# aviadlevis/bhnerf

Hardware: AMD Instinct MI355X
Metric: train ray-samples/sec, 128x128x64-sample image-plane recovery (higher is better)
Workload: dtype bf16

## Files before the change

bhnerf_amd/csrc/fused_bwd128.hip:

```cpp
#include <type_traits>
#include "bwd_common.h"

namespace {

constexpr int MT = 4, KS = 8, TB = 2048;
constexpr int IMG = 32768;
constexpr int OFF_GA = 0, OFF_H = 2 * IMG, OFF_E = 4 * IMG;
constexpr int ENC_IMG = 8192;
constexpr int OFF_DOUT = OFF_E + 2 * ENC_IMG;
constexpr int OFF_DPK = OFF_DOUT + 512;
constexpr int OFF_W0 = OFF_DPK + 256;
constexpr int OFF_B0 = OFF_W0 + 8192;
constexpr int LDS_BYTES = OFF_B0 + 512;
constexpr int CB = (KS + 2) * 1024;
constexpr int SLAB_TILES = 65;
constexpr int SLAB_FLOATS128 = SLAB_TILES * 1024;
constexpr int CPF = 3;

typedef PolBF16 Pol;
typedef Pol::frag frag;

DEVI frag lds_row(const char *smem, unsigned off) { return *reinterpret_cast<const frag *>(smem + off); }
DEVI void lds_put(char *smem, unsigned off, const frag &f) { *reinterpret_cast<frag *>(smem + off) = f; }

DEVI frag tr2(const char *smem, unsigned off_a, unsigned off_b) {
    typedef s16x4 __attribute__((address_space(3))) * lds_v4;
    typedef short s16x8 __attribute__((ext_vector_type(8)));
    const s16x4 lo = __builtin_amdgcn_ds_read_tr16_b64_v4i16((lds_v4)(smem + off_a));
    const s16x4 hi = __builtin_amdgcn_ds_read_tr16_b64_v4i16((lds_v4)(smem + off_b));
    const s16x8 v = __builtin_shufflevector(lo, hi, 0, 1, 2, 3, 4, 5, 6, 7);
    return __builtin_bit_cast(frag, v);
}

DEVI u32x4 make_rsrc(const char *p) {
    const unsigned long long u = reinterpret_cast<unsigned long long>(p);
    const unsigned lo = __builtin_amdgcn_readfirstlane((unsigned)u), hi = __builtin_amdgcn_readfirstlane((unsigned)(u >> 32));
    return u32x4{lo, hi & 0xffffu, 0x7fffffffu, 0x00020000u};
}
#pragma clang diagnostic push
#pragma clang diagnostic ignored "-Winline-asm"
DEVI void dma_piece(const u32x4 &rs, unsigned soff, unsigned lds, unsigned voff) {
    asm volatile("s_mov_b32 m0, %0\n\ts_nop 0\n\tbuffer_load_dwordx4 %1, %2, %3 offen nt lds" ::"s"(lds), "v"(voff), "s"(rs), "s"(soff) : "memory", "m0");
}
#pragma clang diagnostic pop

DEVI unsigned keep_where_nz(unsigned g, unsigned h) {
    typedef short i16x2 __attribute__((ext_vector_type(2)));
    const unsigned sgn = h + 0x7fff7fffu;
    return g & __builtin_bit_cast(unsigned, __builtin_bit_cast(i16x2, sgn) >> (i16x2){15, 15});
}


template <int DEPTH, int SKIPL>
__global__ __launch_bounds__(256) __attribute__((amdgpu_waves_per_eu(1, 1))) void bwd128_kernel(BwdArgs A) {
    static_assert(DEPTH >= 2 && DEPTH <= 4, "14 accumulator tiles per wave at depth 4");
    extern __shared__ __attribute__((aligned(16))) char smem[];
    const FusedArgs &a = A.f;
    clock_stamp(a.clk, BHN_CLK_CHAIN, 0);
    const int tid = threadIdx.x, lane = tid & 63;
    const int wv = __builtin_amdgcn_readfirstlane(tid >> 6);
    const int wi = wv >> 1, wj = wv & 1;
    const int pl = lane & 31, hh = lane >> 5;

    unsigned rowb[2];
    {
        const int swz = ((pl & 3) << 2) | (((pl >> 2) & 3) ^ (pl & 2));
#pragma unroll
        for (int pi = 0; pi < 2; ++pi) rowb[pi] = 256u * (32 * (2 * wj + pi) + pl) + 16u * ((hh ^ swz) & 15);
    }
    const int tg = lane >> 4, tcg = tg & 1, tkh = tg >> 1, tq = (lane & 15) >> 2, tp = lane & 3;
    auto tr_first = [&](int T) -> unsigned {
        const int lc = 2 * tcg + (tp >> 1), swa = (tq << 2) | ((2 * tkh) ^ (tq & 2));
        return 256u * (8 * tkh + tq) + 16u * (((4 * T) ^ lc ^ swa) & 15) + 8u * (tp & 1);
    };
    auto tr_second = [&](int T) -> unsigned {
        const int lc = 2 * tcg + (tp >> 1), swb = (tq << 2) | ((2 * tkh + 1) ^ (tq & 2));
        return 256u * (8 * tkh + tq + 4) + 16u * (((4 * T) ^ lc ^ swb) & 15) + 8u * (tp & 1);
    };
    const unsigned trA_m0 = tr_first(2 * wi), trB_m0 = tr_second(2 * wi), trA_m1 = tr_first(2 * wi + 1), trB_m1 = tr_second(2 * wi + 1);
    const unsigned trA_n0 = tr_first(2 * wj), trB_n0 = tr_second(2 * wj), trA_n1 = tr_first(2 * wj + 1), trB_n1 = tr_second(2 * wj + 1);
    const unsigned trA_w = tr_first(wv), trB_w = tr_second(wv);
    const unsigned trA_me = tr_first(2 * wi + wj), trB_me = tr_second(2 * wi + wj);
    const unsigned trE = 64u * (8 * tkh + tq) + 32u * tcg + 8u * tp;

    const unsigned voffH = 2048u * ((((lane & 15) >> 2) ^ (lane >> 4)) & 3) + 64u * (((lane & 3) ^ wv ^ ((lane >> 4) & 2)) & 3) + 16u * (lane >> 4);
    const unsigned voffE = 16u * ((lane >> 2) & 3) + 64u * (lane & 3) + 256u * (lane >> 4);
    const unsigned lds0 = __builtin_amdgcn_readfirstlane((unsigned)reinterpret_cast<unsigned long long>(smem));

    const long long nquads = A.t.NQ >> 2;
    const long long h_stride = A.t.lin_stride;
    auto dma_h = [&](int l, long long Q, int hb) {
        const u32x4 rs = make_rsrc(A.tape + A.t.h_lin + (long long)l * h_stride + Q * (4ll * MT * TB));
#pragma unroll
        for (int t = 0; t < 8; ++t) {
            const int pb = t >> 1, kk = wv + 4 * (t & 1), k = wv + 4 * t;
            dma_piece(rs, (unsigned)(pb * (MT * TB) + 256 * kk), lds0 + OFF_H + hb * IMG + 1024 * k, voffH);
        }
    };
    auto h_rsrc = [&](int l, long long Q) { return make_rsrc(A.tape + A.t.h_lin + (long long)l * h_stride + Q * (4ll * MT * TB)); };
    auto dma_h_piece = [&](const u32x4 &rs, int hb, int t) {
        const int pb = t >> 1, kk = wv + 4 * (t & 1), k = wv + 4 * t;
        dma_piece(rs, (unsigned)(pb * (MT * TB) + 256 * kk), lds0 + OFF_H + hb * IMG + 1024 * k, voffH);
    };
    auto dma_enc = [&](long long Q, int eb) {
        const u32x4 rs = make_rsrc(A.tape + A.t.enc_off + Q * (4ll * TB));
#pragma unroll
        for (int t = 0; t < 2; ++t) {
            const int e = wv + 4 * t, pb = e >> 1, half = e & 1;
            dma_piece(rs, (unsigned)(pb * TB + 1024 * half), lds0 + OFF_E + eb * ENC_IMG + 1024 * e, voffE);
        }
    };
    const float *dout_g = reinterpret_cast<const float *>(A.tape + A.t.dout_off);
    auto point_dout = [&](long long Q) -> float { return dout_g[(4 * Q + wv) * 32 + pl]; };
    auto put_dout = [&](float d) {
        if (lane < 32) reinterpret_cast<float *>(smem + OFF_DOUT)[32 * wv + pl] = d;
    };
    const unsigned *maskd_g = reinterpret_cast<const unsigned *>(A.tape + A.t.maskd_off);
    auto load_maskd = [&](long long Qx, unsigned (&mw)[2]) {
#pragma unroll
        for (int pi = 0; pi < 2; ++pi) mw[pi] = maskd_g[((4 * Qx + 2 * wj + pi) * 2 + wi) * 64 + lane];
    };
    const __amdgpu_buffer_rsrc_t wrs = __builtin_amdgcn_make_buffer_rsrc(
        const_cast<char *>(a.packed + a.bwd_off + (size_t)(2 * wi) * CB), 0, 0x7fffffff, 0x00020000);
    auto load_w1 = [&](int l, int mi, int ks) -> frag {
        return __builtin_bit_cast(frag, __builtin_amdgcn_raw_buffer_load_b128(wrs, lane * 16, ((l - 1) * MT + mi) * CB + ks * 1024, 0));
    };
    auto load_w = [&](int l, frag (&wf)[2][KS]) {
#pragma unroll
        for (int mi = 0; mi < 2; ++mi)
#pragma unroll
            for (int ks = 0; ks < KS; ++ks) wf[mi][ks] = load_w1(l, mi, ks);
    };
    auto use_w = [&](frag (&wf)[2][KS]) {
#pragma unroll
        for (int mi = 0; mi < 2; ++mi)
#pragma unroll
            for (int ks = 0; ks < KS; ks += 4) asm volatile("" : "+v"(wf[mi][ks]), "+v"(wf[mi][ks + 1]), "+v"(wf[mi][ks + 2]), "+v"(wf[mi][ks + 3]));
    };
    auto drain_and_barrier = [&]() {
        asm volatile("s_waitcnt vmcnt(0) lgkmcnt(0)" ::: "memory");
        __builtin_amdgcn_s_barrier();
        asm volatile("" ::: "memory");
    };

    f32x16 acc[DEPTH - 1][4], acc_e, acc0;
#pragma unroll
    for (int l = 0; l < DEPTH - 1; ++l)
#pragma unroll
        for (int t = 0; t < 4; ++t) { const f32x16 z = {}; acc[l][t] = z; }
    { const f32x16 z = {}; acc_e = z; acc0 = z; }
    float bsum[DEPTH - 1];
#pragma unroll
    for (int l = 0; l < DEPTH - 1; ++l) bsum[l] = 0.f;
    float bout = 0.f;

    auto chain_mma = [&](const frag (&wf)[2][KS], unsigned ga_in, int pi, f32x16 (&c)[2], auto &&side) {
        { const f32x16 z = {}; c[0] = z; c[1] = z; }
        frag bq[CPF + 1];
#pragma unroll
        for (int i = 0; i < CPF; ++i) bq[i] = lds_row(smem, ga_in + (rowb[pi] ^ (32u * i)));
#pragma unroll
        for (int ks = 0; ks < KS; ++ks) {
            if (ks + CPF < KS) bq[(ks + CPF) % (CPF + 1)] = lds_row(smem, ga_in + (rowb[pi] ^ (32u * (ks + CPF))));
            __builtin_amdgcn_sched_barrier(0);
            c[0] = Pol::mma(wf[0][ks], bq[ks % (CPF + 1)], c[0]);
            c[1] = Pol::mma(wf[1][ks], bq[ks % (CPF + 1)], c[1]);
            side(ks);
            __builtin_amdgcn_sched_barrier(0);
        }
        asm volatile("" : "+v"(c[0]), "+v"(c[1]));
    };
    u32x4 ps_hv, ps_hvn, ps_o;
    auto post_off = [&](int pi, int jp) -> unsigned { return rowb[pi] ^ (16u * (4 * (2 * wi + (jp >> 1)) + 2 * (jp & 1))); };
    auto post_begin = [&](int pi, unsigned h_img) { ps_hvn = __builtin_bit_cast(u32x4, lds_row(smem, h_img + post_off(pi, 0))); };
    auto post_slice = [&](const f32x16 (&c)[2], int pi, unsigned h_img, unsigned ga_out, int j) {
        const int mi = j >> 2, s2 = (j >> 1) & 1, half = j & 1;
        if (half == 0) ps_hv = ps_hvn;
        else if (j + 1 < 8) ps_hvn = __builtin_bit_cast(u32x4, lds_row(smem, h_img + post_off(pi, (j + 1) >> 1)));
#pragma unroll
        for (int d = 2 * half; d < 2 * half + 2; ++d) ps_o[d] = keep_where_nz(Pol::pack_a(c[mi][8 * s2 + 2 * d], c[mi][8 * s2 + 2 * d + 1]), ps_hv[d]);
        if (half == 1) lds_put(smem, ga_out + post_off(pi, j >> 1), __builtin_bit_cast(frag, ps_o));
    };
    auto dw_phase = [&](auto enc_tag, unsigned ga_img, unsigned h_img, unsigned e_img, f32x16 (&t)[4], f32x16 &te, float &bs, auto &&side) {
        constexpr bool ENC = decltype(enc_tag)::value;
        struct KF { frag a0, a1, b0, b1, ae, be; };
        auto fetch = [&](int k) {
            KF f;
            const unsigned ko = 4096u * k;
            f.a0 = tr2(smem, ga_img + trA_m0 + ko, ga_img + trB_m0 + ko);
            f.a1 = tr2(smem, ga_img + trA_m1 + ko, ga_img + trB_m1 + ko);
            f.b0 = tr2(smem, h_img + trA_n0 + ko, h_img + trB_n0 + ko);
            f.b1 = tr2(smem, h_img + trA_n1 + ko, h_img + trB_n1 + ko);
            f.ae = tr2(smem, ga_img + trA_me + ko, ga_img + trB_me + ko);
            if constexpr (ENC) f.be = tr2(smem, e_img + trE + 1024u * k, e_img + trE + 1024u * k + 256u);
            else f.be = f.b0;
            return f;
        };
        KF cur = fetch(0);
#pragma unroll
        for (int k = 0; k < 8; ++k) {
            __builtin_amdgcn_sched_barrier(0);
            t[0] = Pol::mma(cur.a0, cur.b0, t[0]);
            t[1] = Pol::mma(cur.a0, cur.b1, t[1]);
            t[2] = Pol::mma(cur.a1, cur.b0, t[2]);
            t[3] = Pol::mma(cur.a1, cur.b1, t[3]);
            if constexpr (ENC) te = Pol::mma(cur.ae, cur.be, te);
            else bs = Pol::sum8(cur.ae, bs);
            if (k + 1 < 8) cur = fetch(k + 1);
            side(k);
            __builtin_amdgcn_sched_barrier(0);
        }
    };
    auto dw0_phase = [&](unsigned ga_img, unsigned e_img, auto &&side) {
        frag af = tr2(smem, ga_img + trA_w, ga_img + trB_w);
        frag be = tr2(smem, e_img + trE, e_img + trE + 256u);
#pragma unroll
        for (int k = 0; k < 8; ++k) {
            frag afn = af, ben = be;
            if (k + 1 < 8) {
                const unsigned ko = 4096u * (k + 1);
                afn = tr2(smem, ga_img + trA_w + ko, ga_img + trB_w + ko);
                ben = tr2(smem, e_img + trE + 1024u * (k + 1), e_img + trE + 1024u * (k + 1) + 256u);
            }
            __builtin_amdgcn_sched_barrier(0);
            acc0 = Pol::mma(af, be, acc0);
            side(k);
            __builtin_amdgcn_sched_barrier(0);
            af = afn; be = ben;
        }
    };
    auto front = [&](const unsigned (&mw)[2], unsigned ga_out) {
#pragma unroll
        for (int pi = 0; pi < 2; ++pi) {
            const float dvp = reinterpret_cast<const float *>(smem + OFF_DOUT)[32 * (2 * wj + pi) + pl];
            const Pol::bf16x2 d2 = {(__bf16)dvp, (__bf16)dvp};
            const unsigned dd = __builtin_bit_cast(unsigned, d2);
#pragma unroll
            for (int mi = 0; mi < 2; ++mi) {
                const unsigned code = mi ? mw[pi] >> 16 : mw[pi];
#pragma unroll
                for (int s2 = 0; s2 < 2; ++s2) {
                    u32x4 o;
#pragma unroll
                    for (int d = 0; d < 4; ++d) {
                        const int lo = (int)(code << (31 - (4 * s2 + d))) >> 31, hi = (int)(code << (31 - (8 + 4 * s2 + d))) >> 31;
                        o[d] = dd & (((unsigned)lo & 0xffffu) | ((unsigned)hi & 0xffff0000u));
                    }
                    lds_put(smem, ga_out + (rowb[pi] ^ (16u * (4 * (2 * wi + mi) + 2 * s2))), __builtin_bit_cast(frag, o));
                }
            }
        }
    };

    for (int i = tid; i < 8192 / 16; i += 256)
        reinterpret_cast<u32x4 *>(smem + OFF_W0)[i] = reinterpret_cast<const u32x4 *>(a.packed + a.fwd_off)[i];
    if (tid < 128) reinterpret_cast<float *>(smem + OFF_B0)[tid] = reinterpret_cast<const float *>(a.packed + a.bias_off)[tid];
    auto make_h1 = [&](unsigned e_img, unsigned h_out) {
        frag eb[2][2], wa[2][2];
#pragma unroll
        for (int pi = 0; pi < 2; ++pi)
#pragma unroll
            for (int ks = 0; ks < 2; ++ks) eb[pi][ks] = lds_row(smem, e_img + 64u * (32 * (2 * wj + pi) + pl) + 16u * (2 * ks + hh));
#pragma unroll
        for (int mi = 0; mi < 2; ++mi)
#pragma unroll
            for (int ks = 0; ks < 2; ++ks) wa[mi][ks] = lds_row(smem, OFF_W0 + 1024u * (2 * (2 * wi + mi) + ks) + 16u * lane);
#pragma unroll
        for (int mi = 0; mi < 2; ++mi) {
            const f32x16 b0 = bias_acc(reinterpret_cast<const float *>(smem + OFF_B0), 2 * wi + mi, hh);
#pragma unroll
            for (int pi = 0; pi < 2; ++pi) {
                f32x16 t = b0;
                t = Pol::mma(wa[mi][0], eb[pi][0], t);
                t = Pol::mma(wa[mi][1], eb[pi][1], t);
                asm volatile("" : "+v"(t));
                frag o[2];
                unsigned unused = 0;
#pragma unroll
                for (int r = 0; r < 16; r += 2) Pol::relu_pair(o[r >> 3], (r & 7) >> 1, r >> 1, t[r], t[r + 1], unused);
#pragma unroll
                for (int s2 = 0; s2 < 2; ++s2) lds_put(smem, h_out + (rowb[pi] ^ (16u * (4 * (2 * wi + mi) + 2 * s2))), o[s2]);
            }
        }
    };

    long long Q = blockIdx.x;
    frag wf[2][KS];
    float dnext = 0.f;
    int eb = 0;
    unsigned mnext[2] = {0u, 0u};
    if (Q < nquads) {
        dma_h(DEPTH - 1, Q, 1);
        dma_enc(Q, 0);
        dnext = point_dout(Q);
        load_maskd(Q, mnext);
        load_w(DEPTH - 1, wf);
        use_w(wf);
        if (lane < 32) bout += dnext;
        put_dout(dnext);
        drain_and_barrier();
        front(mnext, OFF_GA + 0 * IMG);
        drain_and_barrier();
    }
    for (; Q < nquads; Q += gridDim.x) {
#pragma unroll
        for (int l = 0; l < DEPTH - 1; ++l) asm volatile("" : "+a"(acc[l][0]), "+a"(acc[l][1]), "+a"(acc[l][2]), "+a"(acc[l][3]));
        asm volatile("" : "+a"(acc_e), "+a"(acc0));
        const bool has_next = Q + gridDim.x < nquads;
        const long long Qn = has_next ? Q + gridDim.x : Q;
        const unsigned e_img = OFF_E + eb * ENC_IMG;
#pragma unroll
        for (int l = DEPTH - 1; l >= 1; --l) {
            const int gi = (DEPTH - 1 - l) & 1, hi = (DEPTH - l) & 1;
            const unsigned ga_in = OFF_GA + gi * IMG, ga_out = OFF_GA + (gi ^ 1) * IMG, h_img = OFF_H + hi * IMG;
            const u32x4 rs_h = h_rsrc(l - 1 >= 2 ? l - 1 : 2, Q);
            if (l == 2) make_h1(e_img, OFF_H + (hi ^ 1) * IMG);
            if (l == 1) { dnext = point_dout(Qn); load_maskd(Qn, mnext); }
            f32x16 c0[2], c1[2];
            chain_mma(wf, ga_in, 0, c0, [&](int ks) { if (l - 1 >= 2) dma_h_piece(rs_h, hi ^ 1, ks); });
            post_begin(0, h_img);
            chain_mma(wf, ga_in, 1, c1, [&](int ks) { post_slice(c0, 0, h_img, ga_out, ks); });
            post_begin(1, h_img);
            const int ln = (l - 1 >= 1) ? l - 1 : DEPTH - 1;
            auto side_dw = [&](int k) {
                post_slice(c1, 1, h_img, ga_out, k);
                if (k < 4) {
#pragma unroll
                    for (int mi = 0; mi < 2; ++mi) { wf[mi][2 * k] = load_w1(ln, mi, 2 * k); wf[mi][2 * k + 1] = load_w1(ln, mi, 2 * k + 1); }
                }
            };
            if (l == SKIPL) dw_phase(std::true_type{}, ga_in, h_img, e_img, acc[l - 1], acc_e, bsum[l - 1], side_dw);
            else dw_phase(std::false_type{}, ga_in, h_img, e_img, acc[l - 1], acc_e, bsum[l - 1], side_dw);
            use_w(wf);
            if (l == 1) {
                asm volatile("" : "+v"(dnext));
                const float d = has_next ? dnext : 0.f;
                if (lane < 32) bout += d;
                put_dout(d);
            }
            drain_and_barrier();
        }
        {
            const int gi0 = (DEPTH - 1) & 1, hfree = (DEPTH - 1) & 1;
            const u32x4 rs_h = h_rsrc(DEPTH - 1, Qn);
            dma_enc(Qn, eb ^ 1);
            dw0_phase(OFF_GA + gi0 * IMG, e_img, [&](int k) { dma_h_piece(rs_h, hfree, k); });
            front(mnext, OFF_GA + 0 * IMG);
            drain_and_barrier();
        }
        eb ^= 1;
    }
    asm volatile("s_waitcnt vmcnt(0)" ::: "memory");
    float *slab = a.slabs + (long long)blockIdx.x * SLAB_FLOATS128;
    auto flush_tile = [&](int tile, const f32x16 &t) {
        float *tp = slab + (long long)tile * 1024;
#pragma unroll
        for (int g4 = 0; g4 < 4; ++g4) {
            f32x4 v;
#pragma unroll
            for (int e = 0; e < 4; ++e) v[e] = t[4 * g4 + e];
            f32x4 *dst = reinterpret_cast<f32x4 *>(tp + g4 * 256 + lane * 4);
            if (A.accumulate) {
                const f32x4 old = *dst;
#pragma unroll
                for (int e = 0; e < 4; ++e) v[e] += old[e];
            }
            *dst = v;
        }
    };
#pragma unroll
    for (int l = 1; l < DEPTH; ++l) {
        const int base = (l - 1) * 20;
        flush_tile(base + 5 * (2 * wi) + 2 * wj, acc[l - 1][0]);
        flush_tile(base + 5 * (2 * wi) + 2 * wj + 1, acc[l - 1][1]);
        flush_tile(base + 5 * (2 * wi + 1) + 2 * wj, acc[l - 1][2]);
        flush_tile(base + 5 * (2 * wi + 1) + 2 * wj + 1, acc[l - 1][3]);
        if (l == SKIPL) flush_tile(base + 5 * (2 * wi + wj) + 4, acc_e);
        else {
            float v = bsum[l - 1] + __shfl_xor(bsum[l - 1], 32, 64);
            float *tp = slab + (long long)(base + 5 * (2 * wi + wj) + 4) * 1024;
            if (lane < 32) {
                const int row = lane, h2 = (row >> 2) & 1, r = (row & 3) + 4 * (row >> 3);
                float *dst = tp + (r >> 2) * 256 + (31 + 32 * h2) * 4 + (r & 3);
                if (A.accumulate) v += *dst;
                *dst = v;
            }
        }
    }
    flush_tile(60 + wv, acc0);
    {
        float *tp = slab + 64ll * 1024;
        float bs = bout;
#pragma unroll
        for (int o = 16; o > 0; o >>= 1) bs += __shfl_xor(bs, o, 64);
        if (lane == 0) {
            float *dst = tp + 128 + wv;
            if (A.accumulate) bs += *dst;
            *dst = bs;
        }
    }
    clock_stamp(a.clk, BHN_CLK_CHAIN, 1);
}

__global__ __launch_bounds__(256) void dout128_kernel(BwdArgs A) {
    const FusedArgs &a = A.f;
    const long long n = A.t.NQ * 32;
    const float *eg = reinterpret_cast<const float *>(A.tape + A.t.e_off);
    float *dg = reinterpret_cast<float *>(A.tape + A.t.dout_off);
    if (blockIdx.x == 0 && threadIdx.x == 0)
        *reinterpret_cast<unsigned *>(reinterpret_cast<float *>(A.tape + A.t.scratch_off) + 5 * 128) = 0u;
    for (long long i = blockIdx.x * 256ll + threadIdx.x; i < n; i += (long long)gridDim.x * 256) {
        const long long q = i >> 5;
        int b; long long p; bool inb;
        const unsigned qu = (unsigned)q;
        if (A.fwd_nw == 12) tile_point_nw(a, qu / 12u, (int)(qu % 12u), (int)(i & 31), 12, b, p, inb);
        else tile_point_nw(a, qu >> 3, (int)(qu & 7u), (int)(i & 31), 8, b, p, inb);
        const float e = eg[i];
        float d = 0.f;
        if (inb && e != 0.f) {
            const long long ray = a.ray_idx ? (long long)a.ray_idx[p] : (long long)a.fd_G.div((unsigned)p);
            float dE = 0.f;
            for (int s = 0; s < a.Sx; ++s) dE += a.dimages[((long long)b * a.Sx + s) * a.R + ray] * a.w[(long long)s * a.P + p];
            d = dE * e * (1.f - e);
        }
        dg[i] = d;
    }
}

__host__ __device__ inline int virt_feature(int v) { return 16 * ((v >> 4) & 1) + 4 * ((v >> 3) & 1) + (v & 3) + 8 * ((v >> 2) & 1); }

__global__ __launch_bounds__(256) void reduce128_stage1(BwdArgs A, int nslabs, int per) {
    const int tile = blockIdx.x, part = blockIdx.y, s0 = part * per, s1 = (s0 + per < nslabs) ? s0 + per : nslabs;
    if (s0 >= s1) return;
    float *base = A.f.slabs + (long long)tile * 1024 + threadIdx.x * 4;
    f32x4 sum = *reinterpret_cast<const f32x4 *>(base + (long long)s0 * SLAB_FLOATS128);
    for (int wg = s0 + 1; wg < s1; ++wg) {
        const f32x4 v = *reinterpret_cast<const f32x4 *>(base + (long long)wg * SLAB_FLOATS128);
#pragma unroll
        for (int e = 0; e < 4; ++e) sum[e] += v[e];
    }
    *reinterpret_cast<f32x4 *>(base + (long long)s0 * SLAB_FLOATS128) = sum;
}

template <int DEPTH>
__global__ __launch_bounds__(256) void reduce128_kernel(BwdArgs A, int nslabs, int step) {
    const int tile = blockIdx.x, tid = threadIdx.x, g4 = tid >> 6, lane = tid & 63, hh = lane >> 5, col = lane & 31;
    const float *src = A.f.slabs + (long long)tile * 1024 + g4 * 256 + lane * 4;
    f32x4 sum = {0.f, 0.f, 0.f, 0.f};
    for (int wg = 0; wg < nslabs; wg += step) {
        const f32x4 v = *reinterpret_cast<const f32x4 *>(src + (long long)wg * SLAB_FLOATS128);
#pragma unroll
        for (int e = 0; e < 4; ++e) sum[e] += v[e];
    }
    const int WT = A.width_true;
    const float *wout = reinterpret_cast<const float *>(A.f.packed + A.f.wout_off);
    if (tile == 64) {
        if (tid == 32) A.dparams[A.bias_off[DEPTH]] = (sum[0] + sum[1]) + (sum[2] + sum[3]);
        return;
    }
    int l, m, n;
    if (tile >= 60) { l = 0; m = tile - 60; n = 4; }
    else { l = 1 + tile / 20; m = (tile % 20) / 5; n = tile % 5; }
    if (l >= DEPTH) return;
    const bool skip = (A.f.skip_mask >> l) & 1;
    const bool fold = l == DEPTH - 1 && bhn_folds_wout(BHN_BF16, DEPTH);
    if (l == DEPTH - 1) {
        const char *wimg = A.f.packed + A.f.fwd_off + (size_t)(1 + (l - 1) * MT + m) * CB;
        const float *bias = reinterpret_cast<const float *>(A.f.packed + A.f.bias_off) + l * 128;
        float *scr = reinterpret_cast<float *>(A.tape + A.t.scratch_off) + n * 128;
        const int q = n < 4 ? 32 * n + virt_feature(col) : virt_feature(col);
        const int fr = n < 4 ? q >> 4 : KS + (q >> 4), ph = q & 15, h2 = (ph >> 2) & 1, jj = (ph & 3) + 4 * (ph >> 3);
#pragma unroll
        for (int e = 0; e < 4; ++e) {
            const int v = e + 8 * g4 + 4 * hh, i = virt_feature(v);
            float wq;
            if (n == 4 && q == 31) wq = bias[32 * m + i];
            else if (n == 4 && !skip) wq = 0.f;
            else wq = (float)reinterpret_cast<const __bf16 *>(wimg + fr * 1024 + (i + 32 * h2) * 16)[jj];
            float part = wq * sum[e];
#pragma unroll
            for (int o2 = 16; o2 > 0; o2 >>= 1) part += __shfl_xor(part, o2, 64);
            if (col == 0) scr[32 * m + i] = part;
        }
        __shared__ unsigned ticket;
        __threadfence();
        __syncthreads();
        unsigned *count = reinterpret_cast<unsigned *>(reinterpret_cast<float *>(A.tape + A.t.scratch_off) + 5 * 128);
        if (tid == 0) ticket = atomicAdd(count, 1u);
        __syncthreads();
        if (ticket == 4 * 5 - 1) {
            __threadfence();
            const volatile float *all = reinterpret_cast<const volatile float *>(A.tape + A.t.scratch_off);
            if (tid < 128) {
                float s = all[tid];
#pragma unroll
                for (int k = 1; k < 5; ++k) s += all[k * 128 + tid];
                if (tid < WT) A.dparams[A.kernel_off[DEPTH] + tid] = s;
            }
        }
    }
    long long kin = -1;
    bool is_bias = false;
    if (n < 4) {
        const int k = 32 * n + virt_feature(col);
        if (k < WT) kin = k;
    } else {
        const int slot = virt_feature(col);
        if (slot == 31) is_bias = true;
        else {
            const int fe = bhn_enc_slot_feature(slot, A.f.deg);
            if (fe >= 0 && (l == 0 || skip)) kin = (l == 0 ? 0 : WT) + fe;
        }
    }
    if (kin < 0 && !is_bias) return;
#pragma unroll
    for (int e = 0; e < 4; ++e) {
        const int v = e + 8 * g4 + 4 * hh;
        const int o = 32 * m + virt_feature(v);
        if (o >= WT) continue;
        float val = sum[e];
        if (fold) val *= wout[o];
        A.dparams[is_bias ? A.bias_off[l] + o : A.kernel_off[l] + kin * WT + o] = val;
    }
}

}

bool bwd128_supported(int mode, int kernel_width, int depth) {
    return mode == BHN_BF16 && kernel_width == 128 && depth == 4;
}

size_t bwd128_slab_bytes(int grid) { return (size_t)grid * SLAB_FLOATS128 * 4; }

void bwd128_tape_layout(int depth, long long NQ, TapeLayout *t) {
    memset(t, 0, sizeof(*t));
    t->NQ = NQ;
    t->fused128 = 1;
    const long long per_tensor = NQ * (long long)MT * TB;
    long long off = 0;
    t->drop_h1 = 1;
    t->h_off[1] = -1;
    t->drop_hd = 1;
    for (int l = 2; l < depth; ++l) { t->h_off[l] = off; off += per_tensor; }
    t->h_off[depth] = -1;
    t->maskd_off = off; off += NQ * 2ll * 256;
    for (int l = 0; l < depth; ++l) t->ga_off[l] = -1;
    t->lin_stride = per_tensor;
    t->h_lin = -2 * per_tensor;
    t->enc_off = off; off += NQ * (long long)TB;
    t->e_off = off; off += NQ * 128;
    t->dout_off = off; off += NQ * 128;
    t->dout_stride = 128;
    t->mask_off = -1; t->encp_off = -1;
    off = (off + 255) / 256 * 256;
    t->scratch_off = off; off += 5 * 128 * 4 + 256;
    t->total = (long long)(((size_t)off + 1024 + 255) / 256 * 256);
}

int bwd128_launch(const BwdArgs &A, int depth, int grid, hipStream_t st) {
    static DeviceOnce once;
    int dev = 0;
    BHN_HIP(hipGetDevice(&dev));
    BHN_CHECK_DEVICE(dev);
    BHN_HIP(once.run(dev, [&](int &) {
        return hipFuncSetAttribute((const void *)&bwd128_kernel<4, 3>, hipFuncAttributeMaxDynamicSharedMemorySize, 160 * 1024);
    }));
    BHN_CHECK_ARG(depth == 4 && (A.t.NQ & 3) == 0, "fused width-128 backward: depth %d, %lld groups", depth, A.t.NQ);
    {
        long long nb = (A.t.NQ * 32 + 255) / 256;
        if (nb > 4096) nb = 4096;
        hipLaunchKernelGGL(dout128_kernel, dim3((unsigned)nb), dim3(256), 0, st, A);
        BHN_HIP(hipGetLastError());
    }
    hipLaunchKernelGGL((bwd128_kernel<4, 3>), dim3((unsigned)grid), dim3(256), LDS_BYTES, st, A);
    BHN_HIP(hipGetLastError());
    return BHN_OK;
}

int reduce128_launch(const BwdArgs &A, int depth, int nslabs, hipStream_t st) {
    BHN_CHECK_ARG(depth == 4, "fused width-128 backward: depth %d", depth);
    const int parts = 8, per = (nslabs + parts - 1) / parts;
    hipLaunchKernelGGL(reduce128_stage1, dim3(SLAB_TILES, parts), dim3(256), 0, st, A, nslabs, per);
    BHN_HIP(hipGetLastError());
    hipLaunchKernelGGL(reduce128_kernel<4>, dim3(SLAB_TILES), dim3(256), 0, st, A, nslabs, per);
    BHN_HIP(hipGetLastError());
    return BHN_OK;
}
```

bhnerf_amd/csrc/bwd_common.h:

```cpp
#pragma once
#include "fused_common.h"

struct TapeLayout {
    long long NQ;
    long long h_off[BHN_MAX_LAYERS + 1];
    long long ga_off[BHN_MAX_LAYERS];
    long long enc_off, dout_off, mask_off, e_off, total;
    long long h_lin, ga_lin, lin_stride;
    long long encp_off;
    int drop_h1;
    int drop_ga;
    int ga0_chain;
    long long dout_stride;
    int fused128;
    int drop_hd;
    int lbits;
    long long maskd_off, scratch_off;
};

struct BwdArgs {
    FusedArgs f;
    char *tape;
    TapeLayout t;
    int wg_begin[BHN_MAX_LAYERS + 2];
    int accumulate;
    float *dparams;
    long long kernel_off[BHN_MAX_LAYERS + 1], bias_off[BHN_MAX_LAYERS + 1];
    int in_dim[BHN_MAX_LAYERS + 1];
    int F;
    int width_true;
    long long nparams;
    float *t8;
    float *slab0;
    int n_chain_wg;
    int chain_step;
    int fwd_nw;
};


bool bwd128_supported(int mode, int kernel_width, int depth);
size_t bwd128_slab_bytes(int grid);
void bwd128_tape_layout(int depth, long long NQ, TapeLayout *t);
int bwd128_launch(const BwdArgs &A, int depth, int grid, hipStream_t st);
int reduce128_launch(const BwdArgs &A, int depth, int nslabs, hipStream_t st);
```

bhnerf_amd/csrc/fused_bwd.hip:

```cpp
#include <climits>
#include <utility>
#include <type_traits>
#include "fused_common.h"
#include "bwd_common.h"

static constexpr int JOB1_W = 13;
static constexpr int JOBL_W = 7;
static constexpr int GA0C_DIST = 4;
static constexpr int TAPED_DIST = 7;
static constexpr int T8_NBUF = 4;

template <int W, class Pol>
struct BwdGeom {
    static constexpr int MT = W / 32;
    static constexpr int TILE_BYTES = 2 * Pol::FRAG_BYTES;
    static constexpr int TAPE_TILE = Pol::TAPE8 ? 1024 : TILE_BYTES;
    static constexpr int NTMAX = MT + 2;
    static constexpr int SLAB_FLOATS = (MT + 1) * NTMAX * 1024;
    static constexpr int WR = (MT >= 4) ? 4 : MT;
    static constexpr int WC = Pol::NWAVES / WR >= 1 ? Pol::NWAVES / WR : 1;
    static constexpr int WRR = (Pol::NWAVES < WR) ? Pol::NWAVES : WR;
    static constexpr int WCC = Pol::NWAVES / WRR;
    static constexpr int MPW = (MT + WRR - 1) / WRR;
    static constexpr int NPW_ALL = (NTMAX + WCC - 1) / WCC;
// ... 1445 lines not shown
                if (wc == 0) {
#pragma unroll
                    for (int e = 1; e < (WCC > 4 ? 8 : 4); ++e)
                        if (e >= WCC || e * NPW >= nBr) slab[(long long)(MT * BG::NTMAX + m) * 1024 + (lane + 32 * (e >> 2)) * 4 + (e & 3)] = 0.f;
                }
            }
        }
    }
    if constexpr (LAST) {
        float v = bout + __shfl_xor(bout, 32, 64);
        if (out_bias_wave && lane == 0) {
            float *dst = slab + (long long)(MT * BG::NTMAX + MT + (OUTENC ? 1 : 0)) * 1024;
            if (A.accumulate) v += *dst;
            *dst = v;
        }
        if constexpr (OUTENC) {
            float ve = oenc + __shfl_xor(oenc, 32, 64);
            if (out_bias_wave && lane < 32) {
                float *dst = slab + (long long)(MT * BG::NTMAX + MT) * 1024 + lane * 4;
                if (A.accumulate) ve += *dst;
                *dst = ve;
            }
        }
    }
}

template <int W, class Pol>
__global__ __launch_bounds__(Pol::NTHREADS) __attribute__((amdgpu_waves_per_eu(Pol::NWAVES == 4 ? 1 : (W <= 128 ? 4 : 2)))) void dw_kernel(BwdArgs A) {
    extern __shared__ __attribute__((aligned(16))) char smem[];
    const int depth = A.f.depth;
    clock_stamp(A.f.clk, BHN_CLK_DW, 0);
    int job = 0;
    while (job < depth && (int)blockIdx.x >= A.wg_begin[job + 1]) ++job;
    if constexpr (Pol::ELEM_BYTES == 2) {
        const bool out_skip = (A.f.skip_mask >> depth) & 1;
        if (job == depth) {
            if (out_skip) dw_body<W, Pol, JT_OUTSKIP>(A, job, smem);
            else dw_body<W, Pol, JT_OUT>(A, job, smem);
        } else if (job == 0) dw_body2<W, Pol, JT_FIRST>(A, job, smem); else if (job == depth - 1 && A.t.drop_ga) {
            if constexpr (Pol::TAPE8) {
                if ((A.f.skip_mask >> job) & 1) dw_body2<W, Pol, JT_SKIP, true>(A, job, smem);
                else dw_body2<W, Pol, JT_HIDDEN, true>(A, job, smem);
            } else if ((A.f.skip_mask >> job) & 1) {
                if (out_skip) dw_body2<W, Pol, JT_SKIP, true, true>(A, job, smem);
                else dw_body2<W, Pol, JT_SKIP, true>(A, job, smem);
            } else if (A.t.lbits) {
                if (out_skip) dw_body2<W, Pol, JT_HIDDEN, true, true, true>(A, job, smem);
                else dw_body2<W, Pol, JT_HIDDEN, true, false, true>(A, job, smem);
            } else {
                if (out_skip) dw_body2<W, Pol, JT_HIDDEN, true, true>(A, job, smem);
                else dw_body2<W, Pol, JT_HIDDEN, true>(A, job, smem);
            }
        } else if ((A.f.skip_mask >> job) & 1) dw_body2<W, Pol, JT_SKIP>(A, job, smem);
        else if (job == 1 && A.t.drop_h1) dw_body2<W, Pol, JT_HIDDEN1>(A, job, smem);
        else dw_body2<W, Pol, JT_HIDDEN>(A, job, smem);
    } else {
        if (job == depth) {
            if ((A.f.skip_mask >> depth) & 1) dw_body<W, Pol, JT_OUTSKIP>(A, job, smem);
            else dw_body<W, Pol, JT_OUT>(A, job, smem);
        } else if (job == 0) dw_body<W, Pol, JT_FIRST>(A, job, smem);
        else if ((A.f.skip_mask >> job) & 1) dw_body<W, Pol, JT_SKIP>(A, job, smem);
        else dw_body<W, Pol, JT_HIDDEN>(A, job, smem);
    }
    clock_stamp(A.f.clk, BHN_CLK_DW, 1);
}

template <int W, class Pol>
struct ReduceGeom {
    using BG = BwdGeom<W, Pol>;
    static __host__ __device__ int n_b(int l, unsigned skip_mask) { return (l >= 1 ? BG::MT : 0) + ((l == 0 || ((skip_mask >> l) & 1)) ? 1 : 0); }
    static __host__ __device__ int rows(int l, int depth) { return l == depth ? 1 : BG::MT; }
    static __host__ __device__ int blocks(int depth, unsigned skip_mask) {
        int n = 0;
        for (int l = 0; l <= depth; ++l) n += rows(l, depth) * (n_b(l, skip_mask) + 1);
        return n;
    }
};

__global__ __launch_bounds__(256) void chain_slab_stage1(BwdArgs A, int mt, int per) {
    const int tile = blockIdx.x, s0 = blockIdx.y * per, s1 = (s0 + per < A.n_chain_wg) ? s0 + per : A.n_chain_wg;
    if (s0 >= s1) return;
    float *base = A.slab0 + (long long)tile * 1024 + threadIdx.x * 4;
    f32x4 sum = *reinterpret_cast<const f32x4 *>(base + (long long)s0 * mt * 1024);
    for (int wg = s0 + 1; wg < s1; ++wg) {
        const f32x4 v = *reinterpret_cast<const f32x4 *>(base + (long long)wg * mt * 1024);
#pragma unroll
        for (int e = 0; e < 4; ++e) sum[e] += v[e];
    }
    *reinterpret_cast<f32x4 *>(base + (long long)s0 * mt * 1024) = sum;
}

template <int W, class Pol>
__global__ __launch_bounds__(256) void reduce_kernel(BwdArgs A) {
    using BG = BwdGeom<W, Pol>;
    using RG = ReduceGeom<W, Pol>;
    constexpr int MT = BG::MT;
    const int depth = A.f.depth, WT = A.width_true;
    int b = blockIdx.x, l = 0;
    for (; l <= depth; ++l) {
        const int cnt = RG::rows(l, depth) * (RG::n_b(l, A.f.skip_mask) + 1);
        if (b < cnt) break;
        b -= cnt;
    }
    if (l > depth) return;
    const bool has_h = l >= 1, has_enc = (l == 0) || ((A.f.skip_mask >> l) & 1);
    const int nH = has_h ? MT : 0, nB = nH + (has_enc ? 1 : 0);
    const int mi = b / (nB + 1), n = b % (nB + 1);
    const bool out = l == depth, rides = out && A.t.drop_ga;
    const int jl = rides ? depth - 1 : l;
    const int mrow = out ? (rides ? MT : 0) : mi;
    if (!out && 32 * mi >= WT) return;
    const int tid = threadIdx.x, g4 = tid >> 6, lane = tid & 63, hh = lane >> 5, col = lane & 31;
    const float *src = A.f.slabs + (long long)(mrow * BG::NTMAX + n) * 1024 + g4 * 256 + lane * 4;
    f32x4 sum = {0.f, 0.f, 0.f, 0.f};
    const bool from_chain = l == 0 && A.t.ga0_chain;
    if (from_chain) {
        if (n != 0) return;
        const float *s0 = A.slab0 + (long long)mi * 1024 + g4 * 256 + lane * 4;
        for (int wg = 0; wg < A.n_chain_wg; wg += A.chain_step) {
            const f32x4 v = *reinterpret_cast<const f32x4 *>(s0 + (long long)wg * MT * 1024);
#pragma unroll
            for (int e = 0; e < 4; ++e) sum[e] += v[e];
        }
    } else
    for (int wg = A.wg_begin[jl]; wg < A.wg_begin[jl + 1]; ++wg) {
        const f32x4 v = *reinterpret_cast<const f32x4 *>(src + (long long)wg * BG::SLAB_FLOATS);
#pragma unroll
        for (int e = 0; e < 4; ++e) sum[e] += v[e];
    }
    long long kin = -1;
    bool is_bias = false;
    if (n < nH) {
        const int c = (Pol::TAPE8 && !(l == 1 && A.t.drop_h1)) ? t8_feature(n, col) : 32 * n + col;
        if (c < WT) kin = c;
    }
    else if (n < nB) {
        const int fe = bhn_enc_slot_feature(col, A.f.deg);
        if (fe >= 0) kin = (has_h ? WT : 0) + fe;
        else if (from_chain && col == 31) is_bias = true;
    }
    else is_bias = col == 0;
    float lb_tot = (sum[0] + sum[1]) + (sum[2] + sum[3]);
    if constexpr (BG::WCC > 4) lb_tot += __shfl_xor(lb_tot, 32, 64);
    if (kin < 0 && !is_bias) return;
    const int outw = out ? 1 : WT;
#pragma unroll
    for (int e = 0; e < 4; ++e) {
        const int r = 4 * g4 + e, row = (r & 3) + 4 * hh + 8 * (r >> 2);
        const int o = out ? 0 : (Pol::TAPE8 && !from_chain) ? t8_feature(mi, row) : 32 * mi + row;
        if (out ? row != 0 : o >= WT) continue;
        float val = sum[e];
        if (rides && A.t.lbits && n < nH) val = lb_tot;
        A.dparams[is_bias ? A.bias_off[l] + o : A.kernel_off[l] + kin * outw + o] = val;
    }
}

__global__ __launch_bounds__(1024) void t8_dmax_kernel(float *st, const float *dimages, long long n) {
    __shared__ float red[16];
    float m = 0.f;
    for (long long i = blockIdx.x * 1024ll + threadIdx.x; i < n; i += (long long)gridDim.x * 1024) m = __builtin_fmaxf(m, __builtin_fabsf(dimages[i]));
#pragma unroll
    for (int o = 32; o >= 1; o >>= 1) m = __builtin_fmaxf(m, __shfl_xor(m, o, 64));
    if ((threadIdx.x & 63) == 0) red[threadIdx.x >> 6] = m;
    __syncthreads();
    if (threadIdx.x == 0) {
        float d = 0.f;
        for (int i = 0; i < 16; ++i) d = __builtin_fmaxf(d, red[i]);
        if (!(d < __builtin_inff())) d = __builtin_inff();
        atomicMax(reinterpret_cast<unsigned *>(st) + 25, __float_as_uint(d));
    }
}
__global__ void t8_prepare_kernel(float *st, int nl, int fresh) {
    if (threadIdx.x != 0) return;
    float d = st[24];
    if (fresh) {
        d = st[25];
        st[25] = 0.f;
        if (!(d < __builtin_inff())) d = 0.f;
        st[24] = d;
    }
    for (int l = 0; l < nl; ++l) {
        const float a = st[16 + l] * d;
        if (a > 0.f && a < __builtin_inff()) {
            int e;
            const float mant = frexpf(a * (16.f / 448.f), &e);
            if (mant == 0.5f) --e;
            e = e < -100 ? -100 : e > 100 ? 100 : e;
            st[l] = ldexpf(1.f, e);
        } else if (!(st[l] > 0.f && st[l] < __builtin_inff())) st[l] = 1.f;
    }
}
__global__ void t8_update_kernel(float *st, int nl) {
    const int l = threadIdx.x;
    if (l >= nl) return;
    unsigned *bits = reinterpret_cast<unsigned *>(st);
    const float a = __uint_as_float(bits[8 + l]), d = st[24];
    if (a > 0.f && a < __builtin_inff() && d > 0.f) st[16 + l] = a / d;
    bits[8 + l] = 0u;
}
__global__ void t8_open_kernel(float *st) {
    if (threadIdx.x < 8) { st[threadIdx.x] = 0x1p60f; reinterpret_cast<unsigned *>(st)[8 + threadIdx.x] = 0u; }
}

int fused_fill_args(const bhn_model *m, int32_t mode, const void *packed, const bhn_geom *geom,
                    const bhn_frames *fr, bool need_w, FusedArgs *a, MlpShape *s, int nwaves);

static size_t align_up(size_t v, size_t a) { return (v + a - 1) / a * a; }

template <int W, class Pol>
static constexpr bool ga0_chain_ok(int depth) {
    return Pol::ELEM_BYTES == 2 && !Pol::TAPE8 && W / 32 == Pol::NWAVES && depth >= 3;
}
// ... 491 lines not shown
```

Before: 710.3 million.

## Reuse weight-grad A fragment for enc/bias tile and hand-schedule chain MFMAs

```diff
diff --git a/bhnerf_amd/csrc/fused_bwd128.hip b/bhnerf_amd/csrc/fused_bwd128.hip
--- a/bhnerf_amd/csrc/fused_bwd128.hip
+++ b/bhnerf_amd/csrc/fused_bwd128.hip
@@ -44,10 +44,11 @@
 }
 #pragma clang diagnostic pop
 
-DEVI unsigned keep_where_nz(unsigned g, unsigned h) {
+DEVI unsigned keep_where_nz(unsigned g, unsigned h, unsigned one11) {
     typedef short i16x2 __attribute__((ext_vector_type(2)));
-    const unsigned sgn = h + 0x7fff7fffu;
-    return g & __builtin_bit_cast(unsigned, __builtin_bit_cast(i16x2, sgn) >> (i16x2){15, 15});
+    typedef unsigned short u16x2 __attribute__((ext_vector_type(2)));
+    const i16x2 nz = __builtin_elementwise_min(__builtin_bit_cast(i16x2, h), __builtin_bit_cast(i16x2, one11));
+    return __builtin_bit_cast(unsigned, __builtin_bit_cast(u16x2, g) * __builtin_bit_cast(u16x2, nz));
 }
 
 
@@ -61,6 +62,8 @@
     const int wv = __builtin_amdgcn_readfirstlane(tid >> 6);
     const int wi = wv >> 1, wj = wv & 1;
     const int pl = lane & 31, hh = lane >> 5;
+    unsigned one11 = 0x00010001u;
+    asm("" : "+s"(one11));
 
     unsigned rowb[2];
     {
@@ -77,10 +80,10 @@
         const int lc = 2 * tcg + (tp >> 1), swb = (tq << 2) | ((2 * tkh + 1) ^ (tq & 2));
         return 256u * (8 * tkh + tq + 4) + 16u * (((4 * T) ^ lc ^ swb) & 15) + 8u * (tp & 1);
     };
-    const unsigned trA_m0 = tr_first(2 * wi), trB_m0 = tr_second(2 * wi), trA_m1 = tr_first(2 * wi + 1), trB_m1 = tr_second(2 * wi + 1);
+    const int me = 2 * wi + wj, mo = 2 * wi + 1 - wj;
+    const unsigned trA_m0 = tr_first(me), trB_m0 = tr_second(me), trA_m1 = tr_first(mo), trB_m1 = tr_second(mo);
     const unsigned trA_n0 = tr_first(2 * wj), trB_n0 = tr_second(2 * wj), trA_n1 = tr_first(2 * wj + 1), trB_n1 = tr_second(2 * wj + 1);
     const unsigned trA_w = tr_first(wv), trB_w = tr_second(wv);
-    const unsigned trA_me = tr_first(2 * wi + wj), trB_me = tr_second(2 * wi + wj);
     const unsigned trE = 64u * (8 * tkh + tq) + 32u * tcg + 8u * tp;
 
     const unsigned voffH = 2048u * ((((lane & 15) >> 2) ^ (lane >> 4)) & 3) + 64u * (((lane & 3) ^ wv ^ ((lane >> 4) & 2)) & 3) + 16u * (lane >> 4);
@@ -155,7 +158,6 @@
     float bout = 0.f;
 
     auto chain_mma = [&](const frag (&wf)[2][KS], unsigned ga_in, int pi, f32x16 (&c)[2], auto &&side) {
-        { const f32x16 z = {}; c[0] = z; c[1] = z; }
         frag bq[CPF + 1];
 #pragma unroll
         for (int i = 0; i < CPF; ++i) bq[i] = lds_row(smem, ga_in + (rowb[pi] ^ (32u * i)));
@@ -163,12 +165,18 @@
         for (int ks = 0; ks < KS; ++ks) {
             if (ks + CPF < KS) bq[(ks + CPF) % (CPF + 1)] = lds_row(smem, ga_in + (rowb[pi] ^ (32u * (ks + CPF))));
             __builtin_amdgcn_sched_barrier(0);
-            c[0] = Pol::mma(wf[0][ks], bq[ks % (CPF + 1)], c[0]);
-            c[1] = Pol::mma(wf[1][ks], bq[ks % (CPF + 1)], c[1]);
+#pragma unroll
+            for (int mi = 0; mi < 2; ++mi) {
+                if (ks == 0) asm volatile("v_mfma_f32_32x32x16_bf16 %0, %1, %2, 0" : "=&v"(c[mi]) : "v"(wf[mi][ks]), "v"(bq[ks % (CPF + 1)]));
+                else asm volatile("v_mfma_f32_32x32x16_bf16 %0, %1, %2, %0" : "+v"(c[mi]) : "v"(wf[mi][ks]), "v"(bq[ks % (CPF + 1)]));
+            }
             side(ks);
             __builtin_amdgcn_sched_barrier(0);
         }
-        asm volatile("" : "+v"(c[0]), "+v"(c[1]));
+        asm volatile("s_nop 15\n\ts_nop 3" : "+v"(c[0]), "+v"(c[1])
+                     : "v"(bq[0]), "v"(bq[1]), "v"(bq[2]), "v"(bq[3]),
+                       "v"(wf[0][0]), "v"(wf[0][1]), "v"(wf[0][2]), "v"(wf[0][3]), "v"(wf[0][4]), "v"(wf[0][5]), "v"(wf[0][6]), "v"(wf[0][7]),
+                       "v"(wf[1][0]), "v"(wf[1][1]), "v"(wf[1][2]), "v"(wf[1][3]), "v"(wf[1][4]), "v"(wf[1][5]), "v"(wf[1][6]), "v"(wf[1][7]));
     };
     u32x4 ps_hv, ps_hvn, ps_o;
     auto post_off = [&](int pi, int jp) -> unsigned { return rowb[pi] ^ (16u * (4 * (2 * wi + (jp >> 1)) + 2 * (jp & 1))); };
@@ -178,12 +186,12 @@
         if (half == 0) ps_hv = ps_hvn;
         else if (j + 1 < 8) ps_hvn = __builtin_bit_cast(u32x4, lds_row(smem, h_img + post_off(pi, (j + 1) >> 1)));
 #pragma unroll
-        for (int d = 2 * half; d < 2 * half + 2; ++d) ps_o[d] = keep_where_nz(Pol::pack_a(c[mi][8 * s2 + 2 * d], c[mi][8 * s2 + 2 * d + 1]), ps_hv[d]);
+        for (int d = 2 * half; d < 2 * half + 2; ++d) ps_o[d] = keep_where_nz(Pol::pack_a(c[mi][8 * s2 + 2 * d], c[mi][8 * s2 + 2 * d + 1]), ps_hv[d], one11);
         if (half == 1) lds_put(smem, ga_out + post_off(pi, j >> 1), __builtin_bit_cast(frag, ps_o));
     };
     auto dw_phase = [&](auto enc_tag, unsigned ga_img, unsigned h_img, unsigned e_img, f32x16 (&t)[4], f32x16 &te, float &bs, auto &&side) {
         constexpr bool ENC = decltype(enc_tag)::value;
-        struct KF { frag a0, a1, b0, b1, ae, be; };
+        struct KF { frag a0, a1, b0, b1, be; };
         auto fetch = [&](int k) {
             KF f;
             const unsigned ko = 4096u * k;
@@ -191,7 +199,6 @@
             f.a1 = tr2(smem, ga_img + trA_m1 + ko, ga_img + trB_m1 + ko);
             f.b0 = tr2(smem, h_img + trA_n0 + ko, h_img + trB_n0 + ko);
             f.b1 = tr2(smem, h_img + trA_n1 + ko, h_img + trB_n1 + ko);
-            f.ae = tr2(smem, ga_img + trA_me + ko, ga_img + trB_me + ko);
             if constexpr (ENC) f.be = tr2(smem, e_img + trE + 1024u * k, e_img + trE + 1024u * k + 256u);
             else f.be = f.b0;
             return f;
@@ -204,8 +211,8 @@
             t[1] = Pol::mma(cur.a0, cur.b1, t[1]);
             t[2] = Pol::mma(cur.a1, cur.b0, t[2]);
             t[3] = Pol::mma(cur.a1, cur.b1, t[3]);
-            if constexpr (ENC) te = Pol::mma(cur.ae, cur.be, te);
-            else bs = Pol::sum8(cur.ae, bs);
+            if constexpr (ENC) te = Pol::mma(cur.a0, cur.be, te);
+            else bs = Pol::sum8(cur.a0, bs);
             if (k + 1 < 8) cur = fetch(k + 1);
             side(k);
             __builtin_amdgcn_sched_barrier(0);
@@ -371,14 +378,14 @@
 #pragma unroll
     for (int l = 1; l < DEPTH; ++l) {
         const int base = (l - 1) * 20;
-        flush_tile(base + 5 * (2 * wi) + 2 * wj, acc[l - 1][0]);
-        flush_tile(base + 5 * (2 * wi) + 2 * wj + 1, acc[l - 1][1]);
-        flush_tile(base + 5 * (2 * wi + 1) + 2 * wj, acc[l - 1][2]);
-        flush_tile(base + 5 * (2 * wi + 1) + 2 * wj + 1, acc[l - 1][3]);
-        if (l == SKIPL) flush_tile(base + 5 * (2 * wi + wj) + 4, acc_e);
+        flush_tile(base + 5 * me + 2 * wj, acc[l - 1][0]);
+        flush_tile(base + 5 * me + 2 * wj + 1, acc[l - 1][1]);
+        flush_tile(base + 5 * mo + 2 * wj, acc[l - 1][2]);
+        flush_tile(base + 5 * mo + 2 * wj + 1, acc[l - 1][3]);
+        if (l == SKIPL) flush_tile(base + 5 * me + 4, acc_e);
         else {
             float v = bsum[l - 1] + __shfl_xor(bsum[l - 1], 32, 64);
-            float *tp = slab + (long long)(base + 5 * (2 * wi + wj) + 4) * 1024;
+            float *tp = slab + (long long)(base + 5 * me + 4) * 1024;
             if (lane < 32) {
                 const int row = lane, h2 = (row >> 2) & 1, r = (row & 3) + 4 * (row >> 3);
                 float *dst = tp + (r >> 2) * 256 + (31 + 32 * h2) * 4 + (r & 3);
```

After: 710.6 million, median of 2. About the same (+0.0%).

## Fuse two-stage slab reduction into one kernel with last-block handoff and batched loads

Applied to the files above, without the earlier changes.

```diff
diff --git a/bhnerf_amd/csrc/bwd_common.h b/bhnerf_amd/csrc/bwd_common.h
--- a/bhnerf_amd/csrc/bwd_common.h
+++ b/bhnerf_amd/csrc/bwd_common.h
@@ -38,6 +38,24 @@
 };
 
 
+template <int N>
+__device__ __forceinline__ void slab_batch(f32x4 &sum, const float *p, long long stride, int cnt) {
+    f32x4 v[N];
+#pragma unroll
+    for (int k = 0; k < N; ++k) v[k] = *reinterpret_cast<const f32x4 *>(p + (long long)(k < cnt ? k : cnt - 1) * stride);
+#pragma unroll
+    for (int k = 0; k < N; ++k)
+        if (k < cnt) {
+#pragma unroll
+            for (int e = 0; e < 4; ++e) sum[e] += v[k][e];
+        }
+}
+__device__ __forceinline__ void slab_sum(f32x4 &sum, const float *p, long long stride, int n) {
+    for (; n >= 16; n -= 16, p += 16 * stride) slab_batch<16>(sum, p, stride, 16);
+    if (n >= 8) { slab_batch<8>(sum, p, stride, 8); n -= 8; p += 8 * stride; }
+    if (n > 0) slab_batch<8>(sum, p, stride, n);
+}
+
 bool bwd128_supported(int mode, int kernel_width, int depth);
 size_t bwd128_slab_bytes(int grid);
 void bwd128_tape_layout(int depth, long long NQ, TapeLayout *t);
diff --git a/bhnerf_amd/csrc/fused_bwd.hip b/bhnerf_amd/csrc/fused_bwd.hip
--- a/bhnerf_amd/csrc/fused_bwd.hip
+++ b/bhnerf_amd/csrc/fused_bwd.hip
@@ -1551,11 +1551,7 @@
     if (s0 >= s1) return;
     float *base = A.slab0 + (long long)tile * 1024 + threadIdx.x * 4;
     f32x4 sum = *reinterpret_cast<const f32x4 *>(base + (long long)s0 * mt * 1024);
-    for (int wg = s0 + 1; wg < s1; ++wg) {
-        const f32x4 v = *reinterpret_cast<const f32x4 *>(base + (long long)wg * mt * 1024);
-#pragma unroll
-        for (int e = 0; e < 4; ++e) sum[e] += v[e];
-    }
+    slab_sum(sum, base + (long long)(s0 + 1) * mt * 1024, (long long)mt * 1024, s1 - s0 - 1);
     *reinterpret_cast<f32x4 *>(base + (long long)s0 * mt * 1024) = sum;
 }
 
@@ -1586,17 +1582,8 @@
     if (from_chain) {
         if (n != 0) return;
         const float *s0 = A.slab0 + (long long)mi * 1024 + g4 * 256 + lane * 4;
-        for (int wg = 0; wg < A.n_chain_wg; wg += A.chain_step) {
-            const f32x4 v = *reinterpret_cast<const f32x4 *>(s0 + (long long)wg * MT * 1024);
-#pragma unroll
-            for (int e = 0; e < 4; ++e) sum[e] += v[e];
-        }
-    } else
-    for (int wg = A.wg_begin[jl]; wg < A.wg_begin[jl + 1]; ++wg) {
-        const f32x4 v = *reinterpret_cast<const f32x4 *>(src + (long long)wg * BG::SLAB_FLOATS);
-#pragma unroll
-        for (int e = 0; e < 4; ++e) sum[e] += v[e];
-    }
+        slab_sum(sum, s0, (long long)A.chain_step * MT * 1024, (A.n_chain_wg + A.chain_step - 1) / A.chain_step);
+    } else slab_sum(sum, src + (long long)A.wg_begin[jl] * BG::SLAB_FLOATS, BG::SLAB_FLOATS, A.wg_begin[jl + 1] - A.wg_begin[jl]);
     long long kin = -1;
     bool is_bias = false;
     if (n < nH) {
diff --git a/bhnerf_amd/csrc/fused_bwd128.hip b/bhnerf_amd/csrc/fused_bwd128.hip
--- a/bhnerf_amd/csrc/fused_bwd128.hip
+++ b/bhnerf_amd/csrc/fused_bwd128.hip
@@ -15,6 +15,8 @@
 constexpr int CB = (KS + 2) * 1024;
 constexpr int SLAB_TILES = 65;
 constexpr int SLAB_FLOATS128 = SLAB_TILES * 1024;
+constexpr int REDUCE_PARTS = 8;
+constexpr int REDUCE_COUNTERS = 1 + SLAB_TILES;
 constexpr int CPF = 3;
 
 typedef PolBF16 Pol;
@@ -407,8 +409,8 @@
     const long long n = A.t.NQ * 32;
     const float *eg = reinterpret_cast<const float *>(A.tape + A.t.e_off);
     float *dg = reinterpret_cast<float *>(A.tape + A.t.dout_off);
-    if (blockIdx.x == 0 && threadIdx.x == 0)
-        *reinterpret_cast<unsigned *>(reinterpret_cast<float *>(A.tape + A.t.scratch_off) + 5 * 128) = 0u;
+    if (blockIdx.x == 0 && threadIdx.x < REDUCE_COUNTERS)
+        reinterpret_cast<unsigned *>(reinterpret_cast<float *>(A.tape + A.t.scratch_off) + 5 * 128)[threadIdx.x] = 0u;
     for (long long i = blockIdx.x * 256ll + threadIdx.x; i < n; i += (long long)gridDim.x * 256) {
         const long long q = i >> 5;
         int b; long long p; bool inb;
@@ -429,28 +431,54 @@
 
 __host__ __device__ inline int virt_feature(int v) { return 16 * ((v >> 4) & 1) + 4 * ((v >> 3) & 1) + (v & 3) + 8 * ((v >> 2) & 1); }
 
-__global__ __launch_bounds__(256) void reduce128_stage1(BwdArgs A, int nslabs, int per) {
-    const int tile = blockIdx.x, part = blockIdx.y, s0 = part * per, s1 = (s0 + per < nslabs) ? s0 + per : nslabs;
-    if (s0 >= s1) return;
-    float *base = A.f.slabs + (long long)tile * 1024 + threadIdx.x * 4;
-    f32x4 sum = *reinterpret_cast<const f32x4 *>(base + (long long)s0 * SLAB_FLOATS128);
-    for (int wg = s0 + 1; wg < s1; ++wg) {
-        const f32x4 v = *reinterpret_cast<const f32x4 *>(base + (long long)wg * SLAB_FLOATS128);
-#pragma unroll
-        for (int e = 0; e < 4; ++e) sum[e] += v[e];
-    }
-    *reinterpret_cast<f32x4 *>(base + (long long)s0 * SLAB_FLOATS128) = sum;
+typedef float f32x2 __attribute__((ext_vector_type(2)));
+__device__ __forceinline__ void handoff_store(float *p, const f32x4 &v) {
+    using u64 = unsigned long long;
+    __hip_atomic_store(reinterpret_cast<u64 *>(p), __builtin_bit_cast(u64, f32x2{v[0], v[1]}), __ATOMIC_RELAXED, __HIP_MEMORY_SCOPE_AGENT);
+    __hip_atomic_store(reinterpret_cast<u64 *>(p) + 1, __builtin_bit_cast(u64, f32x2{v[2], v[3]}), __ATOMIC_RELAXED, __HIP_MEMORY_SCOPE_AGENT);
+}
+__device__ __forceinline__ f32x4 handoff_load(const float *p) {
+    using u64 = unsigned long long;
+    const f32x2 lo = __builtin_bit_cast(f32x2, __hip_atomic_load(reinterpret_cast<const u64 *>(p), __ATOMIC_RELAXED, __HIP_MEMORY_SCOPE_AGENT));
+    const f32x2 hi = __builtin_bit_cast(f32x2, __hip_atomic_load(reinterpret_cast<const u64 *>(p) + 1, __ATOMIC_RELAXED, __HIP_MEMORY_SCOPE_AGENT));
+    return f32x4{lo[0], lo[1], hi[0], hi[1]};
+}
+__device__ __forceinline__ bool handoff_last(unsigned *count, unsigned n) {
+    __shared__ unsigned ticket;
+    asm volatile("s_waitcnt vmcnt(0)" ::: "memory");
+    __syncthreads();
+    if (threadIdx.x == 0) ticket = atomicAdd(count, 1u);
+    __syncthreads();
+    const bool last = ticket == n - 1;
+    __builtin_amdgcn_fence(__ATOMIC_ACQUIRE, "wavefront");
+    return last;
 }
 
 template <int DEPTH>
-__global__ __launch_bounds__(256) void reduce128_kernel(BwdArgs A, int nslabs, int step) {
-    const int tile = blockIdx.x, tid = threadIdx.x, g4 = tid >> 6, lane = tid & 63, hh = lane >> 5, col = lane & 31;
-    const float *src = A.f.slabs + (long long)tile * 1024 + g4 * 256 + lane * 4;
+__global__ __launch_bounds__(256) void reduce128_kernel(BwdArgs A, int nslabs, int per) {
+    const int tile = blockIdx.x, part = blockIdx.y, tid = threadIdx.x, g4 = tid >> 6, lane = tid & 63, hh = lane >> 5, col = lane & 31;
+    float *src = A.f.slabs + (long long)tile * 1024 + g4 * 256 + lane * 4;
+    unsigned *counters = reinterpret_cast<unsigned *>(reinterpret_cast<float *>(A.tape + A.t.scratch_off) + 5 * 128);
     f32x4 sum = {0.f, 0.f, 0.f, 0.f};
-    for (int wg = 0; wg < nslabs; wg += step) {
-        const f32x4 v = *reinterpret_cast<const f32x4 *>(src + (long long)wg * SLAB_FLOATS128);
-#pragma unroll
-        for (int e = 0; e < 4; ++e) sum[e] += v[e];
+    {
+        const int s0 = part * per, s1 = (s0 + per < nslabs) ? s0 + per : nslabs;
+        if (s1 - s0 > 1) {
+            float *p0 = src + (long long)s0 * SLAB_FLOATS128;
+            f32x4 psum = *reinterpret_cast<const f32x4 *>(p0);
+            slab_sum(psum, p0 + SLAB_FLOATS128, SLAB_FLOATS128, s1 - s0 - 1);
+            handoff_store(p0, psum);
+        }
+        if (!handoff_last(counters + 1 + tile, gridDim.y)) return;
+        const int np = (nslabs + per - 1) / per;
+        f32x4 v[REDUCE_PARTS];
+#pragma unroll
+        for (int k = 0; k < REDUCE_PARTS; ++k) v[k] = handoff_load(src + (long long)(k < np ? k : np - 1) * per * SLAB_FLOATS128);
+#pragma unroll
+        for (int k = 0; k < REDUCE_PARTS; ++k)
+            if (k < np) {
+#pragma unroll
+                for (int e = 0; e < 4; ++e) sum[e] += v[k][e];
+            }
     }
     const int WT = A.width_true;
     const float *wout = reinterpret_cast<const float *>(A.f.packed + A.f.wout_off);
@@ -480,21 +508,14 @@
             float part = wq * sum[e];
 #pragma unroll
             for (int o2 = 16; o2 > 0; o2 >>= 1) part += __shfl_xor(part, o2, 64);
-            if (col == 0) scr[32 * m + i] = part;
-        }
-        __shared__ unsigned ticket;
-        __threadfence();
-        __syncthreads();
-        unsigned *count = reinterpret_cast<unsigned *>(reinterpret_cast<float *>(A.tape + A.t.scratch_off) + 5 * 128);
-        if (tid == 0) ticket = atomicAdd(count, 1u);
-        __syncthreads();
-        if (ticket == 4 * 5 - 1) {
-            __threadfence();
-            const volatile float *all = reinterpret_cast<const volatile float *>(A.tape + A.t.scratch_off);
+            if (col == 0) __hip_atomic_store(scr + 32 * m + i, part, __ATOMIC_RELAXED, __HIP_MEMORY_SCOPE_AGENT);
+        }
+        if (handoff_last(counters, 4 * 5)) {
+            const float *all = reinterpret_cast<const float *>(A.tape + A.t.scratch_off);
             if (tid < 128) {
-                float s = all[tid];
-#pragma unroll
-                for (int k = 1; k < 5; ++k) s += all[k * 128 + tid];
+                float s = __hip_atomic_load(all + tid, __ATOMIC_RELAXED, __HIP_MEMORY_SCOPE_AGENT);
+#pragma unroll
+                for (int k = 1; k < 5; ++k) s += __hip_atomic_load(all + k * 128 + tid, __ATOMIC_RELAXED, __HIP_MEMORY_SCOPE_AGENT);
                 if (tid < WT) A.dparams[A.kernel_off[DEPTH] + tid] = s;
             }
         }
@@ -553,7 +574,8 @@
     t->dout_stride = 128;
     t->mask_off = -1; t->encp_off = -1;
     off = (off + 255) / 256 * 256;
-    t->scratch_off = off; off += 5 * 128 * 4 + 256;
+    t->scratch_off = off; off += 5 * 128 * 4 + 512;
+    static_assert(REDUCE_COUNTERS * 4 <= 512, "the arrival counters of reduce128_kernel outgrow their block");
     t->total = (long long)(((size_t)off + 1024 + 255) / 256 * 256);
 }
 
@@ -579,10 +601,9 @@
 
 int reduce128_launch(const BwdArgs &A, int depth, int nslabs, hipStream_t st) {
     BHN_CHECK_ARG(depth == 4, "fused width-128 backward: depth %d", depth);
-    const int parts = 8, per = (nslabs + parts - 1) / parts;
-    hipLaunchKernelGGL(reduce128_stage1, dim3(SLAB_TILES, parts), dim3(256), 0, st, A, nslabs, per);
-    BHN_HIP(hipGetLastError());
-    hipLaunchKernelGGL(reduce128_kernel<4>, dim3(SLAB_TILES), dim3(256), 0, st, A, nslabs, per);
+    BHN_CHECK_ARG(nslabs >= 1, "fused width-128 backward: %d gradient slabs", nslabs);
+    const int per = (nslabs + REDUCE_PARTS - 1) / REDUCE_PARTS;
+    hipLaunchKernelGGL(reduce128_kernel<4>, dim3(SLAB_TILES, REDUCE_PARTS), dim3(256), 0, st, A, nslabs, per);
     BHN_HIP(hipGetLastError());
     return BHN_OK;
 }
```

New measurement: 712.6 million before, 712.9 million after (median of 2 runs). No clear change (+0.0%).
